# CVMI-Lab/DODA

Measured on AMD Instinct MI355X. Metric: active-voxels/sec fwd+bwd SparseConv U-Net, ScanNet 2cm, higher is better.
Workload: dtype bf16; 1 GPU; cfgs/scannet SparseConv U-Net training step (voxel pooling + fwd + CE + bwd + SGD), 2 cm voxels, 4 scenes/GPU x ~150000 active voxels, random-init weights; global_batch=4, voxels_per_gpu=601279, points_per_gpu=781042, parallelism=dp1, n_classes=20, grad_sync=deferred multi-layer wgrad + bucketed all-reduce, collectives=none (single process), prefetch_gate=off, grad_exchange=no process group

## Files before the change

### doda_amd/csrc/spconv_wgrad.hip

```cpp
#include "wgrad_pairs.hpp"
#include <stdlib.h>
#include <string.h>
#include <mutex>
#include <vector>

typedef float f32x4 __attribute__((ext_vector_type(4)));
typedef short s16x4 __attribute__((ext_vector_type(4)));
typedef __bf16 bf16x8 __attribute__((ext_vector_type(8)));
typedef unsigned int u32x4 __attribute__((ext_vector_type(4)));

namespace {

constexpr int RT = 64;
constexpr int MAX_OGW = 7;
constexpr int PAD = 8;

struct F32 {
    typedef float elem;
    typedef f32x4 frag;
    typedef f32x4 vec;
    static constexpr int VEC = 4;
    static constexpr int KSTEPS = RT / 4;
    typedef float kfrag;
    template <int STRIDE>
// ... 374 lines not shown
    const dim3 grid(total_blocks), block(256);
#define GO(TA, TB, OG)                                                                             \
    do {                                                                                           \
        if (vok) hipLaunchKernelGGL((wgrad_multi_kernel<T, TA, TB, OG, true>), grid, block, 0, s, jobs_dev, n); \
        else hipLaunchKernelGGL((wgrad_multi_kernel<T, TA, TB, OG, false>), grid, block, 0, s, jobs_dev, n); \
    } while (0)
    if (p.OGW == 2) {
        if (p.TA == 3 && p.TB == 3) GO(3, 3, 2);
        else if (p.TA == 1 && p.TB == 1) GO(1, 1, 2);
        else if (p.TA == 2 && p.TB == 1) GO(2, 1, 2);
        else if (p.TA == 1 && p.TB == 2) GO(1, 2, 2);
        else GO(2, 2, 2);
    } else if (p.OGW == 4 && p.TA == 1 && p.TB == 1) GO(1, 1, 4);
    else if (p.OGW == 4 && p.TA == 2 && p.TB == 1) GO(2, 1, 4);
    else if (p.OGW == 4 && p.TA == 1 && p.TB == 2) GO(1, 2, 4);
    else if (p.TA == 1 && p.TB == 1) GO(1, 1, 7);
    else if (p.TA == 2 && p.TB == 1) GO(2, 1, 7);
    else if (p.TA == 1 && p.TB == 2) GO(1, 2, 7);
    else GO(2, 2, 4);
#undef GO
}

struct Staging {
    std::mutex mu;
    void *host = nullptr;
    size_t cap = 0;
    hipEvent_t ev = nullptr;
    int ev_dev = -1;
    bool pending = false;
};
Staging g_staging;
}

enum { J_SKIP = 0, J_ZERO = 1, J_DENSE = 2, J_PAIRS = 3, J_TILE = 4 };

static int wdma_min_rows() {
    static const int v = getenv("DODA_WDMA_MIN_ROWS") ? atoi(getenv("DODA_WDMA_MIN_ROWS")) : 32768;
    return v;
}

static int classify(const doda_wgrad_job &j) {
    if (j.n_rows == 0 && j.dw && j.K > 0 && j.ca > 0 && j.cb > 0)
        return (j.flags & DODA_WGRAD_ACCUMULATE) ? J_SKIP : J_ZERO;
    if (j.tilebook && j.tbl && j.elem_bytes == 2 && j.ca % 16 == 0 && j.ca <= 64 && j.cb % 16 == 0 && j.cb <= 64 &&
        j.K == 27 && j.n_rows > 0 && j.a && j.b && j.dw &&
        j.n_a == j.n_rows && j.ld >= j.n_rows && (size_t)j.n_rows * 128 < 0x7ffffff0ull && (size_t)j.K * j.ld * 4 < 0xffffffffull &&
        !(((uintptr_t)j.a | (uintptr_t)j.b | (uintptr_t)j.tilebook) & 15) && doda_wdma::enabled() &&
        (j.n_rows >= wdma_min_rows() || !doda_pairs::eligible(j)))
        return J_TILE;
    static const bool no_pairs = getenv("DODA_WGRAD_NO_PAIRS") && getenv("DODA_WGRAD_NO_PAIRS")[0] == '1';
    if (doda_pairs::eligible(j) && (!no_pairs || !j.tbl)) return J_PAIRS;
    return J_DENSE;
}

static size_t tile_blocks(const doda_wgrad_job &j) { return (size_t)(j.ca / 16) * (j.cb / 16); }

static bool dense_needs_partial(const JobPlan &jp, const doda_wgrad_job &j) {
    return jp.p.R > 1 || (j.flags & DODA_WGRAD_ACCUMULATE);
}

extern "C" size_t doda_spconv_wgrad_multi_workspace_bytes(const doda_wgrad_job *jobs_h, int32_t n_jobs) {
    if (!jobs_h || n_jobs <= 0) return 0;
    size_t total = 0;
    for (int k = 0; k < n_jobs; ++k) {
        const int cls = classify(jobs_h[k]);
        if (cls == J_PAIRS) { total += doda_pairs::partial_bytes(jobs_h[k]); continue; }
        if (cls == J_TILE) { total += tile_blocks(jobs_h[k]) * align_up(doda_wdma::partial_bytes(jobs_h[k].n_rows), 256); continue; }
        if (cls != J_DENSE) continue;
        JobPlan jp;
        if (!plan_job(jobs_h[k], &jp)) continue;
        if (dense_needs_partial(jp, jobs_h[k])) total += align_up((size_t)jp.p.R * jp.n_elem * 4, 256);
    }
    return total < 256 ? 256 : total;
}

extern "C" size_t doda_spconv_wgrad_multi_desc_bytes(int32_t n_jobs) {
    const size_t per = sizeof(WJob) + sizeof(RJob) > doda_pairs::desc_bytes_per_job()
                           ? sizeof(WJob) + sizeof(RJob) : doda_pairs::desc_bytes_per_job();
    return n_jobs <= 0 ? 0 : align_up((size_t)n_jobs * per + 256, 256);
}

extern "C" int doda_spconv_wgrad_multi(const doda_wgrad_job *jobs_h, int32_t n_jobs, void *ws, size_t ws_bytes,
                                       void *desc_dev, size_t desc_bytes, doda_stream_t stream) {
    if (!jobs_h || n_jobs <= 0 || !ws || !desc_dev) return DODA_ERR_INVALID;
    if (desc_bytes < doda_spconv_wgrad_multi_desc_bytes(n_jobs)) return DODA_ERR_WORKSPACE;
    hipStream_t s = as_stream(stream);
    std::vector<JobPlan> plans(n_jobs);
    std::vector<int> keys, cls(n_jobs), pair_jobs, tile_jobs;
    size_t off = 0;
    for (int k = 0; k < n_jobs; ++k) {
        plans[k].key = -1;
        cls[k] = classify(jobs_h[k]);
        if (cls[k] == J_ZERO) {
            hipMemsetAsync(jobs_h[k].dw, 0, (size_t)jobs_h[k].K * jobs_h[k].ca * jobs_h[k].cb * 4, s);
            continue;
        }
        if (cls[k] == J_SKIP) continue;
        if (cls[k] == J_PAIRS) { pair_jobs.push_back(k); continue; }
        if (cls[k] == J_TILE) { tile_jobs.push_back(k); continue; }
        if (!plan_job(jobs_h[k], &plans[k])) return DODA_ERR_INVALID;
        plans[k].ws_off = off;
        if (dense_needs_partial(plans[k], jobs_h[k])) off += align_up((size_t)plans[k].p.R * plans[k].n_elem * 4, 256);
        bool seen = false;
        for (int key : keys) seen |= key == plans[k].key;
        if (!seen) keys.push_back(plans[k].key);
    }
    doda_pairs::Prepared prep;
    if (!pair_jobs.empty()) {
        const int st = doda_pairs::prepare(jobs_h, pair_jobs.data(), (int)pair_jobs.size(), (char *)ws, &off, &prep);
        if (st != DODA_OK) return st;
    }
    {
        std::vector<char> done(tile_jobs.size(), 0);
        for (size_t q = 0; q < tile_jobs.size(); ++q) {
            if (done[q]) continue;
            const doda_wgrad_job &j0 = jobs_h[tile_jobs[q]];
            std::vector<doda_wdma::Block> blocks;
            for (size_t r = q; r < tile_jobs.size(); ++r) {
                const doda_wgrad_job &j = jobs_h[tile_jobs[r]];
                if (done[r] || j.tilebook != j0.tilebook || j.tbl != j0.tbl || j.n_rows != j0.n_rows || j.ld != j0.ld) continue;
                done[r] = 1;
                const int es = 2;
                for (int ci = 0; ci < j.ca; ci += 16)
                    for (int co = 0; co < j.cb; co += 16)
                        blocks.push_back(doda_wdma::Block{(const char *)j.a + ci * es, (const char *)j.b + co * es,
                                                          j.dw + (size_t)ci * j.cb + co, j.ca * es, j.cb * es, j.ca * j.cb, j.cb,
                                                          (j.flags & DODA_WGRAD_ACCUMULATE) ? 1 : 0});
            }
            const size_t bytes = blocks.size() * align_up(doda_wdma::partial_bytes(j0.n_rows), 256);
            if (ws_bytes < off + bytes) return DODA_ERR_WORKSPACE;
            const int st = doda_wdma::launch(blocks.data(), (int)blocks.size(), j0.tbl, j0.ld, j0.n_rows, j0.tilebook,
                                             (char *)ws + off, s);
            if (st != DODA_OK) return st;
            off += bytes;
        }
    }
    if (ws_bytes < off) return DODA_ERR_WORKSPACE;

    std::vector<WJob> wj;
    std::vector<RJob> rj;
    struct Group { int first, count, blocks, rep; };
    std::vector<Group> groups;
    for (int key : keys) {
        Group g{(int)wj.size(), 0, 0, -1};
        for (int k = 0; k < n_jobs; ++k) {
            if (cls[k] != J_DENSE || plans[k].key != key) continue;
            const doda_wgrad_job &j = jobs_h[k];
            const Plan &p = plans[k].p;
            if (g.rep < 0) g.rep = k;
            WJob d;
            d.a = j.a; d.b = j.b; d.tbl = j.tbl;
            d.out = dense_needs_partial(plans[k], j) ? (float *)((char *)ws + plans[k].ws_off) : j.dw;
            d.ca = j.ca; d.cb = j.cb; d.ld = j.ld; d.K = j.K; d.n_rows = j.n_rows;
            d.rows_per_chunk = p.rows_per_chunk; d.n_tag = p.n_tag; d.n_tbg = p.n_tbg; d.n_og = p.n_og;
            g.blocks += p.R * p.n_tag * p.n_tbg * p.n_og;
            d.blk_end = g.blocks;
            wj.push_back(d);
            ++g.count;
        }
        groups.push_back(g);
    }
    int r_blocks = 0;
    bool scalar_reduce = false;
    for (int k = 0; k < n_jobs; ++k) {
        if (cls[k] != J_DENSE || !dense_needs_partial(plans[k], jobs_h[k])) continue;
        if (plans[k].n_elem % 4 != 0 || (uintptr_t)jobs_h[k].dw % 16 != 0) { scalar_reduce = true; continue; }
        RJob d;
        d.partial = (const float4 *)((char *)ws + plans[k].ws_off);
        d.dw = (float4 *)jobs_h[k].dw;
        d.n_quad = plans[k].n_elem / 4;
        d.R = plans[k].p.R;
        d.accumulate = (jobs_h[k].flags & DODA_WGRAD_ACCUMULATE) ? 1 : 0;
        d.pad = 0;
        int rl = 1;
        while (rl < 16 && rl < d.R) rl *= 2;
        d.pad = rl;
        r_blocks += (int)div_up(d.n_quad, 256 / rl);
        d.blk_end = r_blocks;
        rj.push_back(d);
    }
    const size_t wbytes = wj.size() * sizeof(WJob), rbytes = rj.size() * sizeof(RJob);
    const size_t pair_off = align_up(wbytes + rbytes, 16), pbytes = prep.desc.size();
    const size_t total_desc = pair_off + pbytes;
    if (total_desc > desc_bytes) return DODA_ERR_WORKSPACE;
    if (total_desc > 0) {
        std::lock_guard<std::mutex> lock(g_staging.mu);
        Staging &st = g_staging;
        if (st.pending) { hipEventSynchronize(st.ev); st.pending = false; }
        if (st.cap < total_desc) {
            if (st.host) hipHostFree(st.host);
            st.cap = align_up(total_desc, 4096) * 2;
            if (hipHostMalloc(&st.host, st.cap, hipHostMallocDefault) != hipSuccess) { st.host = nullptr; st.cap = 0; return DODA_ERR_NOMEM; }
        }
        int cur_dev = 0;
        hipGetDevice(&cur_dev);
        if (st.ev && st.ev_dev != cur_dev) { hipEventDestroy(st.ev); st.ev = nullptr; }
        if (!st.ev && hipEventCreateWithFlags(&st.ev, hipEventDisableTiming) != hipSuccess) return DODA_ERR_LAUNCH;
        st.ev_dev = cur_dev;
        if (wbytes) memcpy(st.host, wj.data(), wbytes);
        if (rbytes) memcpy((char *)st.host + wbytes, rj.data(), rbytes);
        if (pbytes) memcpy((char *)st.host + pair_off, prep.desc.data(), pbytes);
        if (hipMemcpyAsync(desc_dev, st.host, total_desc, hipMemcpyHostToDevice, s) != hipSuccess) return DODA_ERR_LAUNCH;
        hipEventRecord(st.ev, s);
        st.pending = true;
    }
    const WJob *wj_dev = (const WJob *)desc_dev;
    for (const Group &g : groups) {
        const JobPlan &jp = plans[g.rep];
        if (jp.esz == 4 && jp.split) launch_multi_variant<F32S>(jp.p, jp.vok, g.blocks, wj_dev + g.first, g.count, s);
        else if (jp.esz == 4) launch_multi_variant<F32>(jp.p, jp.vok, g.blocks, wj_dev + g.first, g.count, s);
        else launch_multi_variant<BF16>(jp.p, jp.vok, g.blocks, wj_dev + g.first, g.count, s);
    }
    int st = doda_check_launch();
    if (st != DODA_OK) return st;
    if (!pair_jobs.empty()) {
        st = doda_pairs::launch(prep, (const char *)desc_dev + pair_off, s);
        if (st != DODA_OK) return st;
    }
    if (!rj.empty()) {
        hipLaunchKernelGGL(wgrad_reduce_multi, dim3(r_blocks), dim3(256), 0, s,
                           (const RJob *)((const char *)desc_dev + wbytes), (int)rj.size());
        st = doda_check_launch();
        if (st != DODA_OK) return st;
    }
    if (scalar_reduce)
        for (int k = 0; k < n_jobs; ++k) {
            if (cls[k] != J_DENSE || !dense_needs_partial(plans[k], jobs_h[k])) continue;
            if (plans[k].n_elem % 4 == 0 && (uintptr_t)jobs_h[k].dw % 16 == 0) continue;
            hipLaunchKernelGGL(wgrad_reduce, dim3(div_up(plans[k].n_elem, 16)), dim3(256), 0, s,
                               (const float *)((char *)ws + plans[k].ws_off), plans[k].p.R, plans[k].n_elem,
                               jobs_h[k].dw, (jobs_h[k].flags & DODA_WGRAD_ACCUMULATE) ? 1 : 0);
        }
    return doda_check_launch();
}
```

### doda_amd/csrc/wgrad_pairs.hpp

```cpp
#pragma once
#include "common.hpp"
#include <vector>

namespace doda_pairs {

bool eligible(const doda_wgrad_job &j);

size_t partial_bytes(const doda_wgrad_job &j);

struct Prepared {
    std::vector<unsigned char> desc;
    struct Group { int ta, tb, first, count, blocks; };
    std::vector<Group> groups;
    size_t reduce_off = 0;
    int n_reduce = 0, reduce_blocks = 0;
};

int prepare(const doda_wgrad_job *jobs, const int *which, int n, char *ws_base, size_t *ws_off, Prepared *out);

int launch(const Prepared &p, const void *desc_dev, hipStream_t s);

size_t desc_bytes_per_job();

}

namespace doda_wdma {
bool enabled();
void set_enabled(bool on);
int max_jobs();
size_t partial_bytes(int n_rows);
struct Block { const void *x, *dy; float *dw; int x_stride, dy_stride, ldo, ldc, accumulate; };
int launch(const Block *blocks, int n_blocks, const int32_t *tbl, int ld, int n_rows, const void *tilebook, void *part,
           hipStream_t s);
}
```

### doda_amd/csrc_ext/doda_torch.cpp

```cpp
#include <torch/extension.h>
#include <torch/csrc/autograd/engine.h>
#include <torch/csrc/autograd/function.h>
#include <torch/csrc/autograd/functions/utils.h>
#include <torch/csrc/autograd/graph_task.h>
#include <torch/csrc/autograd/saved_variable.h>
#include <c10/hip/HIPGuard.h>
#include <unordered_map>
#include <c10/hip/HIPStream.h>
#include <c10/hip/HIPCachingAllocator.h>
#include <hip/hip_runtime_api.h>

#include <cstring>
#include <functional>
#include <mutex>
#include <vector>

#include "../../include/doda_hip.h"
#include <chrono>
#include <cstdlib>

static const bool g_poison = [] { const char *e = getenv("DODA_POISON"); return e && e[0] == '1'; }();
static inline at::Tensor poisoned(at::Tensor t) {
    if (g_poison && t.defined() && t.is_cuda() && t.numel() > 0)
        (void)hipMemsetAsync(t.data_ptr(), 0xFF, (size_t)t.numel() * t.element_size(), c10::hip::getCurrentHIPStream(t.device().index()).stream());
// ... 274 lines not shown
}

bool read_back_blocking(const void *dev_ptr, int32_t *out, int n, void *st, int dev) {
    static const bool spin = getenv("DODA_SPIN_READBACK") && getenv("DODA_SPIN_READBACK")[0] == '1';
    if (spin) return false;
    struct Slot { int32_t *host = nullptr; hipEvent_t ev = nullptr; int dev = -1; };
    static thread_local Slot slot;
    const int cur = dev;
    c10::hip::HIPGuard dev_guard((c10::DeviceIndex)dev);
    if (!slot.host)
        TORCH_CHECK(hipHostMalloc((void **)&slot.host, 64, hipHostMallocDefault) == hipSuccess, "doda: hipHostMalloc");
    if (!slot.ev || slot.dev != cur) {
        if (slot.ev) (void)hipEventDestroy(slot.ev);
        slot.ev = nullptr;
        TORCH_CHECK(hipEventCreateWithFlags(&slot.ev, hipEventBlockingSync | hipEventDisableTiming) == hipSuccess, "doda: hipEventCreate");
        slot.dev = cur;
    }
    TORCH_CHECK(hipMemcpyAsync(slot.host, dev_ptr, (size_t)n * 4, hipMemcpyDeviceToHost, (hipStream_t)st) == hipSuccess, "doda: hipMemcpyAsync");
    TORCH_CHECK(hipEventRecord(slot.ev, (hipStream_t)st) == hipSuccess, "doda: hipEventRecord");
    TORCH_CHECK(hipEventSynchronize(slot.ev) == hipSuccess, "doda: hipEventSynchronize");
    for (int k = 0; k < n; ++k) out[k] = slot.host[k];
    return true;
}
int32_t read_back_i32(const at::Tensor &t, void *st) {
    int32_t v = 0;
    if (read_back_blocking(t.data_ptr(), &v, 1, st, (int)t.device().index())) return v;
    return t.item<int32_t>();
}

typedef std::tuple<at::Tensor, at::Tensor, at::Tensor, at::Tensor, std::vector<int64_t>, at::Tensor, at::Tensor,
                   at::Tensor, at::Tensor, at::Tensor, at::Tensor> PyramidLevel;
std::vector<PyramidLevel> build_pyramid(const at::Tensor &indices_in, std::vector<int64_t> shape, int64_t batch,
                                        int64_t n_levels, int64_t pairs_min_rows, int64_t tile_min_rows,
                                        int64_t tile_levels) {
    TORCH_CHECK(indices_in.is_cuda() && indices_in.scalar_type() == at::kInt && indices_in.dim() == 2 &&
                indices_in.size(1) == 4 && shape.size() == 3, "doda build_pyramid: indices must be int32 [M,4] on the GPU");
    std::vector<PyramidLevel> out;
    at::Tensor indices = indices_in.contiguous();
    const auto iopt = indices.options();
    void *st = stream_of(indices);
    for (int64_t lvl = 0; lvl < n_levels; ++lvl) {
        const int32_t m = (int32_t)indices.size(0);
        int32_t shp[3] = {(int32_t)shape[0], (int32_t)shape[1], (int32_t)shape[2]};
        size_t wsb = doda_rulebook_workspace_bytes(m);
        {
            const long double cells = (long double)batch * shape[0] * shape[1] * shape[2];
            static const long long grid_max = [] {
                const char *e = getenv("DODA_RULEBOOK_GRID_MAX_LOG2");
                const int b = e ? atoi(e) : 28;
                return 1ll << (b < 0 ? 0 : b > 30 ? 30 : b);
            }();
            if (m > 0 && cells > 0 && cells <= (long double)grid_max) wsb = (wsb + 255) / 256 * 256 + (size_t)cells * 4;
        }
        at::Tensor ws = pempty({(int64_t)(wsb > 256 ? wsb : 256)}, iopt.dtype(at::kByte));
        const bool tiled = lvl < tile_levels && tile_min_rows >= 0 && m >= tile_min_rows;
        at::Tensor nbr = tiled ? table_with_tilebook(27, m, iopt) : pempty({27, m}, iopt);
        check(doda_rulebook_subm((const int32_t *)indices.data_ptr(), m, shp, (int32_t)batch, 3,
                                 (int32_t *)nbr.data_ptr(), m, ws.data_ptr(), (size_t)ws.numel(), st),
              "doda_rulebook_subm");
        if (tiled) build_tilebook(nbr, st);
        at::Tensor sp, sn, sh, dp, dn, dh;
        const bool with_pairs = pairs_min_rows >= 0 && m >= pairs_min_rows;
        const bool subm_pairs = with_pairs && !tiled;
        if (subm_pairs) std::tie(sp, sn, sh) = export_pairs(nbr, m, true, st);
        if (lvl == n_levels - 1) {
            out.emplace_back(nbr, at::Tensor(), at::Tensor(), at::Tensor(), std::vector<int64_t>(), sp, sn, sh, dp, dn, dh);
            break;
        }
        at::Tensor parent = pempty({m > 0 ? m : 1}, iopt), off = pempty({m > 0 ? m : 1}, iopt);
        at::Tensor out_idx = pempty({m > 0 ? m : 1, 4}, iopt), count = pempty({1}, iopt);
        check(doda_rulebook_down2_assign((const int32_t *)indices.data_ptr(), m, shp, (int32_t)batch,
                                         (int32_t *)parent.data_ptr(), (int32_t *)off.data_ptr(),
                                         (int32_t *)out_idx.data_ptr(), (int32_t *)count.data_ptr(), ws.data_ptr(),
                                         (size_t)ws.numel(), st), "doda_rulebook_down2_assign");
        const int32_t m_out = read_back_i32(count, st);
        at::Tensor child = pempty({8, m_out}, iopt), par_off = pempty({8, m}, iopt);
        check(doda_rulebook_down2_tables((const int32_t *)parent.data_ptr(), (const int32_t *)off.data_ptr(), m, m_out,
                                         (int32_t *)child.data_ptr(), m_out, (int32_t *)par_off.data_ptr(), m, st),
              "doda_rulebook_down2_tables");
        static const bool down_pairs = [] { const char *e = getenv("DODA_WGRAD_PAIRS_DOWN"); return e && e[0] == '1'; }();
        if (with_pairs && down_pairs) std::tie(dp, dn, dh) = export_pairs(par_off, m, false, st);
        std::vector<int64_t> oshape = {(shape[0] - 2) / 2 + 1, (shape[1] - 2) / 2 + 1, (shape[2] - 2) / 2 + 1};
        at::Tensor outids = out_idx.narrow(0, 0, m_out);
        out.emplace_back(nbr, outids, child, par_off, oshape, sp, sn, sh, dp, dn, dh);
        indices = outids;
        shape = oshape;
    }
    return out;
// ... 1261 lines not shown
                                  pair_in, pair_out, pair_num, pair_seg, true);
        return std::make_pair(r[0], r[1].defined() ? c10::optional<at::Tensor>(r[1]) : c10::nullopt);
    }, "sparse conv that also returns the BatchNorm statistics partials of its output",
          py::arg("features"), py::arg("weight"), py::arg("fwd_tbl"), py::arg("bwd_tbl"), py::arg("n_out"),
          py::arg("bwd_layout"), py::arg("pk_fwd"), py::arg("pk_bwd"), py::arg("residual"),
          py::arg("pair_in") = py::none(), py::arg("pair_out") = py::none(), py::arg("pair_num") = py::none(),
          py::arg("pair_seg") = py::none());
    m.def("residual_block", [](const at::Tensor &x, const c10::optional<at::Tensor> &stats_in, const std::vector<at::Tensor> &bn1,
                               const std::vector<at::Tensor> &bn2, bool training, double momentum1, double eps1,
                               double momentum2, double eps2, const std::vector<c10::optional<at::Tensor>> &cv1,
                               const std::vector<c10::optional<at::Tensor>> &cv2,
                               const std::vector<c10::optional<at::Tensor>> &rb, int64_t n_out,
                               const c10::optional<at::Tensor> &skip, bool want_stats,
                               const std::vector<c10::optional<at::Tensor>> &sc, const c10::optional<at::Tensor> &stats_in_b) {
        auto r = residual_block(x, stats_in, bn1, bn2, training, momentum1, eps1, momentum2, eps2, cv1, cv2, rb, n_out, skip,
                                want_stats, sc, stats_in_b);
        return std::make_pair(r[0], r[1].defined() ? c10::optional<at::Tensor>(r[1]) : c10::nullopt);
    }, "BatchNorm -> ReLU -> SubM conv -> BatchNorm -> ReLU -> SubM conv (+ skip) in one call",
          py::arg("x"), py::arg("stats_in"), py::arg("bn1"), py::arg("bn2"), py::arg("training"), py::arg("momentum1"),
          py::arg("eps1"), py::arg("momentum2"), py::arg("eps2"), py::arg("cv1"), py::arg("cv2"), py::arg("rb"),
          py::arg("n_out"), py::arg("skip"), py::arg("want_stats"),
          py::arg("sc") = std::vector<c10::optional<at::Tensor>>(), py::arg("stats_in_b") = py::none());
    m.def("set_bn_fusion", [](bool on) { g_bn_fusion = on; }, "BatchNorm statistics in the conv epilogues (default on)");
    m.def("gather", [](const at::Tensor &x, const at::Tensor &w, const c10::optional<at::Tensor> &packed,
                       const at::Tensor &tbl, int64_t n_out, int64_t layout, int64_t nc, bool out_f32) {
        return gather(x, w, packed, tbl, n_out, layout, nc, out_f32);
    }, "raw gather-GEMM");
    m.def("wgrad", [](const at::Tensor &a, const at::Tensor &b, const at::Tensor &tbl, int64_t n_rows) {
        return wgrad(a, b, tbl, n_rows);
    }, "raw weight gradient");
    m.def("build_pyramid", &build_pyramid,
          "all SubM k3 and k2s2 rulebooks of an n-level U-Net in one call (13 native builds, 6 size read-backs)",
          py::arg("indices"), py::arg("shape"), py::arg("batch"), py::arg("n_levels"), py::arg("pairs_min_rows") = -1,
          py::arg("tile_min_rows") = -1, py::arg("tile_levels") = 2,
          py::call_guard<py::gil_scoped_release>());
    m.def("build_pyramid_probe", [](const at::Tensor &indices, std::vector<int64_t> shape, int64_t batch, int64_t n_levels,
                                    int64_t pairs_min_rows, int64_t tile_min_rows, int64_t tile_levels) {
              auto levels = build_pyramid(indices, shape, batch, n_levels, pairs_min_rows, tile_min_rows, tile_levels);
              int64_t nt = -1, o64 = 0, o32 = 0;
              if (!levels.empty()) {
                  const at::Tensor &tbl = std::get<0>(levels[0]);
                  const void *tb = tilebook_behind(tbl, tbl.dim() == 2 ? tbl.size(1) : 0);
                  if (tb) {
                      const int64_t T = doda_tilebook_tile(), K = tbl.size(0), UMAX = doda_tilebook_umax();
                      nt = (tbl.size(1) + T - 1) / T;
                      (void)K; (void)UMAX; (void)nt;
                      char *p = (char *)const_cast<void *>(tb) + doda_tilebook_bytes((int32_t)tbl.size(1), (int32_t)tbl.size(0)) - 8;
                      int32_t ov[2] = {0, 0};
                      if (!read_back_blocking(p, ov, 2, stream_of(tbl), (int)tbl.device().index())) {
                          at::Tensor over = at::from_blob(p, {2}, tbl.options()).cpu();
                          ov[0] = over[0].item<int32_t>();
                          ov[1] = over[1].item<int32_t>();
                      }
                      o64 = ov[0];
                      o32 = ov[1];
                  }
              }
              return std::make_tuple(levels, nt, o64, o32);
          }, py::arg("indices"), py::arg("shape"), py::arg("batch"), py::arg("n_levels"), py::arg("pairs_min_rows") = -1,
          py::arg("tile_min_rows") = -1, py::arg("tile_levels") = 2, py::call_guard<py::gil_scoped_release>());
    m.def("with_tilebook", [](const at::Tensor &tbl) {
              TORCH_CHECK(tbl.is_cuda() && tbl.scalar_type() == at::kInt && tbl.dim() == 2, "doda with_tilebook: int32 [K, M] table");
              at::Tensor out = table_with_tilebook(tbl.size(0), tbl.size(1), tbl.options());
              out.copy_(tbl);
              if (tilebook_behind(out, out.size(1))) build_tilebook(out, stream_of(out));
              return out;
          }, "copy of a gather table with its tilebook (doda_tilebook_build) in the same storage");
    m.def("has_tilebook", [](const at::Tensor &tbl) { return tilebook_behind(tbl, tbl.dim() == 2 ? tbl.size(1) : 0) != nullptr; });
    m.def("tilebook_parts", [](const at::Tensor &tbl) {
              const void *tb = tilebook_behind(tbl, tbl.size(1));
              TORCH_CHECK(tb, "doda tilebook_parts: no tilebook");
              const int64_t T = doda_tilebook_tile(), nt = (tbl.size(1) + T - 1) / T, K = tbl.size(0), UMAX = doda_tilebook_umax();
              TORCH_CHECK(K == 27 && T == 256, "doda tilebook_parts: layout of csrc/tilebook.hpp");
              const int64_t LW = 10;
              char *p = (char *)const_cast<void *>(tb);
              auto o32 = tbl.options();
              at::Tensor order = pempty({UMAX}, at::TensorOptions().dtype(at::kLong));
              for (int64_t e = 0; e < UMAX; ++e) order.data_ptr<int64_t>()[e] = (((e >> 5) & 7) * 32 + (e & 31)) * 4 + (e >> 8);
              at::Tensor ulist = at::from_blob(p, {nt, UMAX}, o32).index_select(1, order.to(tbl.device()));
              at::Tensor pos = pempty({T}, at::TensorOptions().dtype(at::kLong));
              for (int64_t t = 0; t < T; ++t) pos.data_ptr<int64_t>()[t] = (t & 0xC0) | (((t & 3) | ((t & 4) << 1) | ((t & 8) >> 1)) << 2) | ((t >> 4) & 3);
              at::Tensor words = at::from_blob(p + nt * UMAX * 4, {nt, LW, T}, o32).to(at::kLong).index_select(2, pos.to(tbl.device()));
              std::vector<at::Tensor> per_offset;
              for (int64_t o = 0; o < K; ++o)
                  per_offset.push_back(words.select(1, (o & 1) * 5 + (o >> 1) / 3).bitwise_right_shift(10 * ((o >> 1) % 3)).bitwise_and(0x3ff));
              at::Tensor lidx = at::stack(per_offset, 1).to(at::kShort);
              at::Tensor ucount = at::from_blob(p + nt * UMAX * 4 + nt * T * LW * 4, {nt}, o32).clone();
              return std::make_tuple(ulist, lidx, ucount);
          });
    m.def("tilebook_overflow", [](const at::Tensor &tbl) {
              const void *tb = tilebook_behind(tbl, tbl.size(1));
              TORCH_CHECK(tb, "doda tilebook_overflow: no tilebook");
              const int64_t T = doda_tilebook_tile(), nt = (tbl.size(1) + T - 1) / T, K = tbl.size(0), UMAX = doda_tilebook_umax();
// ... 86 lines not shown
```

### doda_amd/spconv/ops.py

```python
import os

import numpy as np

import torch

from .. import ops as _ops
from .._ext import ext as _ext
from .core import IndiceData

PAIRS_MIN_ROWS = 65536
WGRAD_PAIRS_DOWN = os.environ.get("DODA_WGRAD_PAIRS_DOWN", "0") == "1"


def _triple(v):
    if isinstance(v, (list, tuple, np.ndarray)):
        out = [int(x) for x in v]
        if len(out) != 3:
            raise ValueError("expected 3 values, got %r" % (v,))
        return out
    return [int(v)] * 3


def get_conv_output_size(input_size, kernel_size, stride, padding, dilation):
    out = []
# ... 11 lines not shown
        tbl = _ops.rulebook_subm(indices, spatial_shape, batch_size, k[0])
    else:
        tbl = _ops.rulebook_subm_generic(indices, spatial_shape, batch_size, k)
    return IndiceData("subm", indices, indices, list(spatial_shape), list(spatial_shape), tbl)


def build_down2(indices, batch_size, spatial_shape, ksize, stride, padding, dilation):
    k, s, p, d = _triple(ksize), _triple(stride), _triple(padding), _triple(dilation)
    if k != [2, 2, 2] or s != [2, 2, 2] or p != [0, 0, 0] or d != [1, 1, 1]:
        if k[0] * k[1] * k[2] > 27:
            raise NotImplementedError("doda_amd SparseConv3d supports kernel volumes <= 27, got k=%r" % (k,))
        outids, tbl, tbl_rev, out_shape = _ops.rulebook_conv(indices, spatial_shape, batch_size, k, s, p, d)
        return IndiceData("down2", outids, indices, list(spatial_shape), out_shape, tbl, tbl_rev)
    outids, child, par_off, out_shape = _ops.rulebook_down2(indices, spatial_shape, batch_size)
    return IndiceData("down2", outids, indices, list(spatial_shape), out_shape, child, par_off)


def get_indice_pairs(indices, batch_size, spatial_shape, ksize=3, stride=1, padding=0, dilation=1,
                     out_padding=0, subm=False, transpose=False, grid=None, use_hash=False):
    if transpose:
        raise NotImplementedError("transposed sparse convolution is not part of DODA's path")
    if subm:
        data = build_subm(indices, batch_size, spatial_shape, ksize)
    else:
        data = build_down2(indices, batch_size, spatial_shape, ksize, stride, padding, dilation)
    return data.outids, data.indice_pairs, data.indice_pair_num


TILE_MIN_ROWS = 32768
TILE_KERNEL = os.environ.get("DODA_NO_TILE", "0") != "1"
TILE_OVERFLOW_MAX = 0.25
TILE_BACKOFF = 64
_tile_state = {"skip": 0, "last": None}


def build_pyramid(tensor, n_levels, subm_key="subm%d", down_key="spconv%d", first_level=1, with_pairs=False,
                  with_tiles=None):
    indices, shape = tensor.indices, tensor.spatial_shape
    n_tile_levels = (2 if with_pairs else 0) if with_tiles is None else (2 if with_tiles is True else int(with_tiles))
    if (_ext is not None and not tensor.indice_dict and indices.is_cuda and indices.dtype == torch.int32
            and indices.shape[0] > 0 and all(int(v) >= 2 for v in shape)):
        tiles_on = TILE_KERNEL and n_tile_levels > 0
        if tiles_on and _tile_state["skip"] > 0:
            _tile_state["skip"] -= 1
            tiles_on = False
        levels, nt, over64, over32 = _ext.build_pyramid_probe(indices, [int(v) for v in shape], int(tensor.batch_size),
                                                              int(n_levels), PAIRS_MIN_ROWS if with_pairs else -1,
                                                              TILE_MIN_ROWS if tiles_on else -1, n_tile_levels)
        if tiles_on and nt >= 0:
            _tile_state["last"] = (nt, over64, over32)
            if over32 > TILE_OVERFLOW_MAX * nt:
                _tile_state["skip"] = TILE_BACKOFF
                levels = [((lv[0].clone() if _ext.has_tilebook(lv[0]) else lv[0]),) + tuple(lv[1:]) for lv in levels]
        for k, (nbr, outids, child, par_off, oshape, sp, sn, sh, dp, dn, dh) in enumerate(levels):
            lvl = first_level + k
            data = tensor.indice_dict[subm_key % lvl] = IndiceData("subm", indices, indices, list(shape),
                                                                   list(shape), nbr)
            if sp is not None:
                data._wpairs = (sp, sn, sh)
            if k == len(levels) - 1:
                break
            data = tensor.indice_dict[down_key % lvl] = IndiceData("down2", outids, indices, list(shape),
                                                                   list(oshape), child, par_off)
            if dp is not None:
                data._wpairs = (dp, dn, dh)
            indices, shape = outids, list(oshape)
        return tensor.indice_dict
    for lvl in range(first_level, first_level + n_levels):
        key = subm_key % lvl
        if key not in tensor.indice_dict:
            tensor.indice_dict[key] = build_subm(indices, tensor.batch_size, shape, 3)
        if (with_pairs and indices.shape[0] >= PAIRS_MIN_ROWS
                and not (_ext is not None and _ext.has_tilebook(tensor.indice_dict[key].tbl))):
            tensor.indice_dict[key].wgrad_lists()
        if lvl == first_level + n_levels - 1:
            break
        key = down_key % lvl
        data = tensor.indice_dict.get(key)
        if data is None:
            data = build_down2(indices, tensor.batch_size, shape, 2, 2, 0, 1)
            tensor.indice_dict[key] = data
        if with_pairs and WGRAD_PAIRS_DOWN and indices.shape[0] >= PAIRS_MIN_ROWS:
            data.wgrad_lists()
        indices, shape = data.outids, data.out_spatial_shape
    return tensor.indice_dict
```

Measured before the change: 132.9 million voxels/s.

## Add wide-channel tilebook weight-gradient kernel for deeper U-Net levels

Adds a new wgrad path (J_WIDE) for subm layers with wider channels that are not pair-eligible. It uses 1024-thread workgroups that stage dy and gathered x rows per 256-row tile in LDS, run all 27 offsets across 16 waves with bf16 MFMA, write per-chunk partials, and reduce them in a second kernel. The pyramid builder now also attaches tilebooks to deeper levels (default up to 7) so these layers can use the tile-list gather instead of the dense per-offset path. Building extra tilebooks costs more time during rulebook construction, and the partial buffers plus the separate reduce launch add memory traffic.

```diff
diff --git a/doda_amd/csrc/spconv_wgrad.hip b/doda_amd/csrc/spconv_wgrad.hip
--- a/doda_amd/csrc/spconv_wgrad.hip
+++ b/doda_amd/csrc/spconv_wgrad.hip
@@ -430,7 +430,7 @@
 Staging g_staging;
 }
 
-enum { J_SKIP = 0, J_ZERO = 1, J_DENSE = 2, J_PAIRS = 3, J_TILE = 4 };
+enum { J_SKIP = 0, J_ZERO = 1, J_DENSE = 2, J_PAIRS = 3, J_TILE = 4, J_WIDE = 5 };
 
 static int wdma_min_rows() {
     static const int v = getenv("DODA_WDMA_MIN_ROWS") ? atoi(getenv("DODA_WDMA_MIN_ROWS")) : 32768;
@@ -440,6 +440,7 @@
 static int classify(const doda_wgrad_job &j) {
     if (j.n_rows == 0 && j.dw && j.K > 0 && j.ca > 0 && j.cb > 0)
         return (j.flags & DODA_WGRAD_ACCUMULATE) ? J_SKIP : J_ZERO;
+    if (doda_wwide::eligible(j) && !doda_pairs::eligible(j)) return J_WIDE;
     if (j.tilebook && j.tbl && j.elem_bytes == 2 && j.ca % 16 == 0 && j.ca <= 64 && j.cb % 16 == 0 && j.cb <= 64 &&
         j.K == 27 && j.n_rows > 0 && j.a && j.b && j.dw &&
         j.n_a == j.n_rows && j.ld >= j.n_rows && (size_t)j.n_rows * 128 < 0x7ffffff0ull && (size_t)j.K * j.ld * 4 < 0xffffffffull &&
@@ -451,6 +452,12 @@
     return J_DENSE;
 }
 
+static std::vector<int> wide_chunks(const doda_wgrad_job *jobs_h, const std::vector<int> &idx) {
+    std::vector<int> rpc;
+    for (int k : idx) rpc.push_back(make_plan(jobs_h[k].K, jobs_h[k].ca, jobs_h[k].cb, jobs_h[k].n_rows, 2, true).rows_per_chunk);
+    return rpc;
+}
+
 static size_t tile_blocks(const doda_wgrad_job &j) { return (size_t)(j.ca / 16) * (j.cb / 16); }
 
 static bool dense_needs_partial(const JobPlan &jp, const doda_wgrad_job &j) {
@@ -460,8 +467,10 @@
 extern "C" size_t doda_spconv_wgrad_multi_workspace_bytes(const doda_wgrad_job *jobs_h, int32_t n_jobs) {
     if (!jobs_h || n_jobs <= 0) return 0;
     size_t total = 0;
+    std::vector<int> wide_jobs;
     for (int k = 0; k < n_jobs; ++k) {
         const int cls = classify(jobs_h[k]);
+        if (cls == J_WIDE) { wide_jobs.push_back(k); continue; }
         if (cls == J_PAIRS) { total += doda_pairs::partial_bytes(jobs_h[k]); continue; }
         if (cls == J_TILE) { total += tile_blocks(jobs_h[k]) * align_up(doda_wdma::partial_bytes(jobs_h[k].n_rows), 256); continue; }
         if (cls != J_DENSE) continue;
@@ -469,12 +478,15 @@
         if (!plan_job(jobs_h[k], &jp)) continue;
         if (dense_needs_partial(jp, jobs_h[k])) total += align_up((size_t)jp.p.R * jp.n_elem * 4, 256);
     }
+    const std::vector<int> rpc = wide_chunks(jobs_h, wide_jobs);
+    total += doda_wwide::partial_bytes(jobs_h, wide_jobs.data(), rpc.data(), (int)wide_jobs.size());
     return total < 256 ? 256 : total;
 }
 
 extern "C" size_t doda_spconv_wgrad_multi_desc_bytes(int32_t n_jobs) {
-    const size_t per = sizeof(WJob) + sizeof(RJob) > doda_pairs::desc_bytes_per_job()
-                           ? sizeof(WJob) + sizeof(RJob) : doda_pairs::desc_bytes_per_job();
+    size_t per = sizeof(WJob) + sizeof(RJob) > doda_pairs::desc_bytes_per_job()
+                     ? sizeof(WJob) + sizeof(RJob) : doda_pairs::desc_bytes_per_job();
+    if (per < doda_wwide::desc_bytes_per_job()) per = doda_wwide::desc_bytes_per_job();
     return n_jobs <= 0 ? 0 : align_up((size_t)n_jobs * per + 256, 256);
 }
 
@@ -484,7 +496,7 @@
     if (desc_bytes < doda_spconv_wgrad_multi_desc_bytes(n_jobs)) return DODA_ERR_WORKSPACE;
     hipStream_t s = as_stream(stream);
     std::vector<JobPlan> plans(n_jobs);
-    std::vector<int> keys, cls(n_jobs), pair_jobs, tile_jobs;
+    std::vector<int> keys, cls(n_jobs), pair_jobs, tile_jobs, wide_jobs;
     size_t off = 0;
     for (int k = 0; k < n_jobs; ++k) {
         plans[k].key = -1;
@@ -496,6 +508,7 @@
         if (cls[k] == J_SKIP) continue;
         if (cls[k] == J_PAIRS) { pair_jobs.push_back(k); continue; }
         if (cls[k] == J_TILE) { tile_jobs.push_back(k); continue; }
+        if (cls[k] == J_WIDE) { wide_jobs.push_back(k); continue; }
         if (!plan_job(jobs_h[k], &plans[k])) return DODA_ERR_INVALID;
         plans[k].ws_off = off;
         if (dense_needs_partial(plans[k], jobs_h[k])) off += align_up((size_t)plans[k].p.R * plans[k].n_elem * 4, 256);
@@ -533,6 +546,16 @@
             off += bytes;
         }
     }
+    std::vector<unsigned char> wide_desc;
+    int wide_wgs = 0, wide_red = 0;
+    if (!wide_jobs.empty()) {
+        const std::vector<int> rpc = wide_chunks(jobs_h, wide_jobs);
+        const size_t bytes = doda_wwide::partial_bytes(jobs_h, wide_jobs.data(), rpc.data(), (int)wide_jobs.size());
+        if (ws_bytes < off + bytes) return DODA_ERR_WORKSPACE;
+        doda_wwide::prepare(jobs_h, wide_jobs.data(), rpc.data(), (int)wide_jobs.size(), (char *)ws + off, wide_desc, &wide_wgs,
+                            &wide_red);
+        off += bytes;
+    }
     if (ws_bytes < off) return DODA_ERR_WORKSPACE;
 
     std::vector<WJob> wj;
@@ -579,7 +602,8 @@
     }
     const size_t wbytes = wj.size() * sizeof(WJob), rbytes = rj.size() * sizeof(RJob);
     const size_t pair_off = align_up(wbytes + rbytes, 16), pbytes = prep.desc.size();
-    const size_t total_desc = pair_off + pbytes;
+    const size_t wide_off = align_up(pair_off + pbytes, 16), wdbytes = wide_desc.size();
+    const size_t total_desc = wide_off + wdbytes;
     if (total_desc > desc_bytes) return DODA_ERR_WORKSPACE;
     if (total_desc > 0) {
         std::lock_guard<std::mutex> lock(g_staging.mu);
@@ -598,6 +622,7 @@
         if (wbytes) memcpy(st.host, wj.data(), wbytes);
         if (rbytes) memcpy((char *)st.host + wbytes, rj.data(), rbytes);
         if (pbytes) memcpy((char *)st.host + pair_off, prep.desc.data(), pbytes);
+        if (wdbytes) memcpy((char *)st.host + wide_off, wide_desc.data(), wdbytes);
         if (hipMemcpyAsync(desc_dev, st.host, total_desc, hipMemcpyHostToDevice, s) != hipSuccess) return DODA_ERR_LAUNCH;
         hipEventRecord(st.ev, s);
         st.pending = true;
@@ -613,6 +638,10 @@
     if (st != DODA_OK) return st;
     if (!pair_jobs.empty()) {
         st = doda_pairs::launch(prep, (const char *)desc_dev + pair_off, s);
+        if (st != DODA_OK) return st;
+    }
+    if (!wide_jobs.empty()) {
+        st = doda_wwide::launch((const char *)desc_dev + wide_off, (int)wide_jobs.size(), wide_wgs, wide_red, s);
         if (st != DODA_OK) return st;
     }
     if (!rj.empty()) {
diff --git a/doda_amd/csrc/spconv_wwide.hip b/doda_amd/csrc/spconv_wwide.hip
--- /dev/null
+++ b/doda_amd/csrc/spconv_wwide.hip
@@ -0,0 +1,313 @@
+#include "common.hpp"
+#include "tilebook.hpp"
+#include "wgrad_pairs.hpp"
+#include <stdlib.h>
+#include <string.h>
+#include <algorithm>
+#include <vector>
+
+namespace {
+
+typedef float f32x4w __attribute__((ext_vector_type(4)));
+typedef short s16x4w __attribute__((ext_vector_type(4)));
+typedef __bf16 bf16x8w __attribute__((ext_vector_type(8)));
+typedef unsigned int u32x4w __attribute__((ext_vector_type(4)));
+
+constexpr int WW_WAVES = 16;
+constexpr int WW_MO = (TB_K + WW_WAVES - 1) / WW_WAVES;
+constexpr int WW_MAX_BLOCKS = 9;
+constexpr int WW_MAX_TA = 3, WW_MAX_TB = 7;
+constexpr int WW_LIST_BYTES = TB_UMAX * 4;
+constexpr int ww_stage_bytes(int ta, int tb) { return TB_T * 32 * tb + (TB_LMAX + 1) * 32 * ta; }
+constexpr int WW_STAGE_MAX = ww_stage_bytes(3, 3);
+constexpr int WW_SMEM = WW_LIST_BYTES + TB_LIDX_BYTES + WW_STAGE_MAX;
+static_assert(WW_SMEM <= 160 * 1024, "one workgroup per CU");
+static_assert(TB_T + 1 <= TB_LMAX + 1, "the dense fallback stages 256 rows into the row slots");
+
+struct WwJob {
+    const unsigned short *x, *dy;
+    const int32_t *tbl;
+    const void *tb;
+    float *dw, *part;
+    int ca, cb, ld, n_rows, nt, ta, tb_, n_sb, P, rpc, accumulate;
+    int wg_end, red_end;
+    int pad;
+};
+
+template <class J>
+__device__ __forceinline__ int ww_find(const J *jobs, int n, int blk, bool red) {
+    int lo = 0, hi = n - 1;
+    while (lo < hi) {
+        const int mid = (lo + hi) >> 1;
+        if (blk < (red ? jobs[mid].red_end : jobs[mid].wg_end)) hi = mid; else lo = mid + 1;
+    }
+    return lo;
+}
+
+__device__ __forceinline__ s16x4w ww_tr(unsigned addr) {
+    return __builtin_amdgcn_ds_read_tr16_b64_v4i16((__attribute__((address_space(3))) s16x4w *)(uintptr_t)addr);
+}
+__device__ __forceinline__ bf16x8w ww_frag(unsigned a_lo, unsigned a_hi) {
+    const s16x4w lo = ww_tr(a_lo), hi = ww_tr(a_hi);
+    return __builtin_bit_cast(bf16x8w, __builtin_shufflevector(lo, hi, 0, 1, 2, 3, 4, 5, 6, 7));
+}
+
+template <int TA, int TB>
+__device__ void ww_body(const WwJob &d, int local, unsigned char *smem) {
+    constexpr int RA = 32 * TA, RB = 32 * TB;
+    constexpr int CIS = 16 * TA, COS = 16 * TB, SLICE = TB_K * CIS * COS;
+    const int tid = threadIdx.x, wid = __builtin_amdgcn_readfirstlane(tid >> 6);
+    const int lane = tid & 63, i = lane & 15, g = lane >> 4, q4 = i >> 2, c4 = i & 3;
+    const int slice = local / d.P, p = local - slice * d.P;
+    const int sa = slice / d.n_sb, sb = slice - sa * d.n_sb;
+    const int ca0 = sa * CIS, cb0 = sb * COS;
+    const int r_begin = p * d.rpc, r_end = min(d.n_rows, r_begin + d.rpc);
+    const int tile_begin = r_begin / TB_T, tile_end = (r_end - 1) / TB_T + 1;
+    static_assert(ww_stage_bytes(TA, TB) <= WW_STAGE_MAX, "staging buffers");
+    const int32_t *tb_ulist = (const int32_t *)d.tb;
+    const uint32_t *tb_lidx = (const uint32_t *)(tb_ulist + (size_t)d.nt * TB_UMAX);
+    const int32_t *tb_ucount = (const int32_t *)(tb_lidx + (size_t)d.nt * (TB_LIDX_BYTES / 4));
+
+    int32_t *list_s = reinterpret_cast<int32_t *>(smem);
+    const unsigned *lidx_s = reinterpret_cast<const unsigned *>(smem + WW_LIST_BYTES);
+    unsigned char *dy_s = smem + WW_LIST_BYTES + TB_LIDX_BYTES;
+    unsigned char *rows_s = dy_s + TB_T * RB;
+    const unsigned dy_base = (unsigned)(uintptr_t)dy_s, rows_base = (unsigned)(uintptr_t)rows_s;
+
+    f32x4w acc[WW_MO][TA][TB];
+#pragma unroll
+    for (int m = 0; m < WW_MO; ++m)
+#pragma unroll
+        for (int a = 0; a < TA; ++a)
+#pragma unroll
+            for (int b = 0; b < TB; ++b) acc[m][a][b] = (f32x4w){0.f, 0.f, 0.f, 0.f};
+
+    auto multiply = [&](bool dense, int only_o, int ks_begin, int ks_end) {
+#pragma unroll 1
+        for (int ks = ks_begin; ks < ks_end; ++ks) {
+            const int r = 32 * ks + 8 * g + q4;
+            bf16x8w bf[TB];
+#pragma unroll
+            for (int b = 0; b < TB; ++b) {
+                const unsigned a0 = dy_base + (unsigned)(r * RB + b * 32 + c4 * 8);
+                bf[b] = ww_frag(a0, a0 + 4u * RB);
+            }
+#pragma unroll
+            for (int m = 0; m < WW_MO; ++m) {
+                const int o = wid + WW_WAVES * m;
+                if (o >= TB_K || (dense && o != only_o)) continue;
+                unsigned s0, s1;
+                if (dense) {
+                    s0 = (unsigned)(r + 1);
+                    s1 = (unsigned)(r + 5);
+                } else {
+                    const unsigned *pl = lidx_s + tb_lplane(o) * TB_T;
+                    const unsigned sh = tb_lshift(o);
+                    s0 = __builtin_amdgcn_ubfe(pl[tb_lpos(r)], sh, 10u);
+                    s1 = __builtin_amdgcn_ubfe(pl[tb_lpos(r + 4)], sh, 10u);
+                }
+                const unsigned x0 = rows_base + s0 * RA + (unsigned)(c4 * 8), x1 = rows_base + s1 * RA + (unsigned)(c4 * 8);
+#pragma unroll
+                for (int a = 0; a < TA; ++a) {
+                    const bf16x8w af = ww_frag(x0 + 32u * a, x1 + 32u * a);
+#pragma unroll
+                    for (int b = 0; b < TB; ++b)
+                        acc[m][a][b] = __builtin_amdgcn_mfma_f32_16x16x32_bf16(af, bf[b], acc[m][a][b], 0, 0, 0);
+                }
+            }
+        }
+    };
+
+    for (int e = tid; e < RA / 16; e += 1024) reinterpret_cast<u32x4w *>(rows_s)[e] = (u32x4w){0u, 0u, 0u, 0u};
+    for (int tile = tile_begin; tile < tile_end; ++tile) {
+        const int t0 = tile * TB_T;
+        const int ks_begin = max(0, (r_begin - t0) / 32), ks_end = min(TB_T / 32, (r_end - t0 + 31) / 32);
+        const int ucount = tb_ucount[tile];
+        const bool listed = ucount <= TB_LMAX;
+        if (listed) {
+            const int e = (tid & 3) * 256 + ((tid >> 7) & 7) * 32 + ((tid >> 2) & 31);
+            list_s[e] = tb_ulist[(size_t)tile * TB_UMAX + tid];
+            for (int v = tid; v < TB_LIDX_BYTES / 16; v += 1024)
+                reinterpret_cast<u32x4w *>(smem + WW_LIST_BYTES)[v] =
+                    reinterpret_cast<const u32x4w *>(tb_lidx + (size_t)tile * (TB_LIDX_BYTES / 4))[v];
+        }
+        for (int v = tid; v < TB_T * (RB / 16); v += 1024) {
+            const int t = v / (RB / 16), f = v - t * (RB / 16);
+            u32x4w val = (u32x4w){0u, 0u, 0u, 0u};
+            if (t0 + t < d.n_rows) val = *reinterpret_cast<const u32x4w *>(d.dy + (size_t)(t0 + t) * d.cb + cb0 + f * 8);
+            *reinterpret_cast<u32x4w *>(dy_s + t * RB + f * 16) = val;
+        }
+        doda_sync();
+        if (listed) {
+            for (int v = tid; v < ucount * (RA / 16); v += 1024) {
+                const int e = v / (RA / 16), f = v - e * (RA / 16);
+                const int row = list_s[e];
+                *reinterpret_cast<u32x4w *>(rows_s + (e + 1) * RA + f * 16) =
+                    *reinterpret_cast<const u32x4w *>(d.x + (size_t)row * d.ca + ca0 + f * 8);
+            }
+            doda_sync();
+            multiply(false, 0, ks_begin, ks_end);
+            doda_sync();
+        } else {
+            for (int o = 0; o < TB_K; ++o) {
+                for (int v = tid; v < TB_T * (RA / 16); v += 1024) {
+                    const int t = v / (RA / 16), f = v - t * (RA / 16);
+                    const int row = t0 + t < d.n_rows ? d.tbl[(size_t)o * d.ld + t0 + t] : -1;
+                    u32x4w val = (u32x4w){0u, 0u, 0u, 0u};
+                    if (row >= 0) val = *reinterpret_cast<const u32x4w *>(d.x + (size_t)row * d.ca + ca0 + f * 8);
+                    *reinterpret_cast<u32x4w *>(rows_s + (t + 1) * RA + f * 16) = val;
+                }
+                doda_sync();
+                multiply(true, o, ks_begin, ks_end);
+                doda_sync();
+            }
+        }
+    }
+
+    float *dst = d.part + (size_t)local * SLICE;
+#pragma unroll
+    for (int m = 0; m < WW_MO; ++m) {
+        const int o = wid + WW_WAVES * m;
+        if (o >= TB_K) continue;
+#pragma unroll
+        for (int a = 0; a < TA; ++a)
+#pragma unroll
+            for (int b = 0; b < TB; ++b)
+#pragma unroll
+                for (int r = 0; r < 4; ++r)
+                    dst[((size_t)o * CIS + a * 16 + 4 * g + r) * COS + b * 16 + i] = acc[m][a][b][r];
+    }
+}
+
+#define WW_SHAPES(X) X(3, 3) X(2, 4) X(2, 3) X(1, 5) X(1, 6) X(1, 7) X(1, 4) X(1, 3)
+
+__global__ __launch_bounds__(1024) void wgrad_wide(const WwJob *__restrict__ jobs, int n_jobs) {
+    __shared__ __attribute__((aligned(16))) unsigned char smem[WW_SMEM];
+    const int j = ww_find(jobs, n_jobs, (int)blockIdx.x, false);
+    const WwJob d = jobs[j];
+    const int local = (int)blockIdx.x - (j == 0 ? 0 : jobs[j - 1].wg_end);
+#define WW_CASE(A, B) if (d.ta == A && d.tb_ == B) { ww_body<A, B>(d, local, smem); return; }
+    WW_SHAPES(WW_CASE)
+#undef WW_CASE
+}
+
+__global__ __launch_bounds__(256) void wgrad_wide_reduce(const WwJob *__restrict__ jobs, int n_jobs) {
+    __shared__ float4 part[256];
+    const int j = ww_find(jobs, n_jobs, (int)blockIdx.x, true);
+    const WwJob d = jobs[j];
+    const int blk = (int)blockIdx.x - (j == 0 ? 0 : jobs[j - 1].red_end);
+    int RL = 1;
+    while (RL < 16 && RL < d.P) RL *= 2;
+    const int EL = 256 / RL, el = (int)threadIdx.x % EL, rl = (int)threadIdx.x / EL;
+    const long long q = (long long)blk * EL + el, n_quad = (long long)TB_K * d.ca * d.cb / 4;
+    const int CIS = 16 * d.ta, COS = 16 * d.tb_, SLICE = TB_K * CIS * COS;
+    const float *src = nullptr;
+    if (q < n_quad) {
+        const long long e = 4 * q;
+        const int co = (int)(e % d.cb), ci = (int)((e / d.cb) % d.ca), o = (int)(e / ((long long)d.ca * d.cb));
+        const int slice = (ci / CIS) * d.n_sb + co / COS;
+        src = d.part + ((size_t)slice * d.P) * SLICE + ((size_t)o * CIS + ci % CIS) * COS + co % COS;
+    }
+    float4 s = make_float4(0.f, 0.f, 0.f, 0.f);
+    if (src)
+        for (int r = rl; r < d.P; r += RL) {
+            const float4 v = *reinterpret_cast<const float4 *>(src + (size_t)r * SLICE);
+            s.x += v.x; s.y += v.y; s.z += v.z; s.w += v.w;
+        }
+    part[rl * EL + el] = s;
+    doda_sync();
+    if (rl == 0 && src) {
+        float4 t = part[el];
+        for (int r = 1; r < RL; ++r) {
+            const float4 v = part[r * EL + el];
+            t.x += v.x; t.y += v.y; t.z += v.z; t.w += v.w;
+        }
+        float4 *dst = reinterpret_cast<float4 *>(d.dw) + q;
+        if (d.accumulate) {
+            const float4 old = *dst;
+            t.x += old.x; t.y += old.y; t.z += old.z; t.w += old.w;
+        }
+        *dst = t;
+    }
+}
+
+bool ww_shape(int ca, int cb, int *ta, int *tb) {
+    const int A = ca / 16, B = cb / 16;
+    int b = B;
+    while (b > WW_MAX_TB || B % b) --b;
+    int a = WW_MAX_TA;
+    while (a > 1 && (A % a || a * b > WW_MAX_BLOCKS)) --a;
+    bool known = false;
+#define WW_KNOWN(X, Y) known |= (a == X && b == Y);
+    WW_SHAPES(WW_KNOWN)
+#undef WW_KNOWN
+    *ta = a; *tb = b;
+    return known;
+}
+
+}
+
+namespace doda_wwide {
+
+bool eligible(const doda_wgrad_job &j) {
+    int ta, tb;
+    return j.tilebook && j.tbl && j.elem_bytes == 2 && j.K == TB_K && j.n_rows > 0 && j.a && j.b && j.dw &&
+           j.ca % 16 == 0 && j.cb % 16 == 0 && j.ca >= 48 && j.cb >= 48 && j.ca <= 224 && j.cb <= 224 &&
+           j.n_a == j.n_rows && j.ld >= j.n_rows && !(((uintptr_t)j.a | (uintptr_t)j.b | (uintptr_t)j.tilebook | (uintptr_t)j.dw) & 15) &&
+           ww_shape(j.ca, j.cb, &ta, &tb);
+}
+
+struct Plan { std::vector<int> order; std::vector<WwJob> d; int wgs = 0, red_blocks = 0; size_t part_bytes = 0; };
+
+static Plan plan(const doda_wgrad_job *jobs, const int *idx, const int *rows_per_chunk, int n) {
+    Plan pl;
+    for (int k = 0; k < n; ++k) pl.order.push_back(k);
+    std::stable_sort(pl.order.begin(), pl.order.end(), [&](int a, int b) { return jobs[idx[a]].n_rows > jobs[idx[b]].n_rows; });
+    for (int kk : pl.order) {
+        const doda_wgrad_job &j = jobs[idx[kk]];
+        WwJob d;
+        d.x = (const unsigned short *)j.a; d.dy = (const unsigned short *)j.b; d.tbl = j.tbl; d.tb = j.tilebook;
+        d.dw = j.dw; d.part = nullptr;
+        d.ca = j.ca; d.cb = j.cb; d.ld = j.ld; d.n_rows = j.n_rows; d.nt = (j.n_rows + TB_T - 1) / TB_T;
+        ww_shape(j.ca, j.cb, &d.ta, &d.tb_);
+        d.n_sb = j.cb / (16 * d.tb_);
+        d.rpc = rows_per_chunk[kk];
+        d.P = (j.n_rows + d.rpc - 1) / d.rpc;
+        d.accumulate = (j.flags & DODA_WGRAD_ACCUMULATE) ? 1 : 0;
+        const int slices = (j.ca / (16 * d.ta)) * d.n_sb;
+        d.part = (float *)(uintptr_t)pl.part_bytes;
+        pl.part_bytes += align_up((size_t)slices * d.P * TB_K * 256 * d.ta * d.tb_ * 4, 256);
+        pl.wgs += slices * d.P;
+        d.wg_end = pl.wgs;
+        int rl = 1;
+        while (rl < 16 && rl < d.P) rl *= 2;
+        pl.red_blocks += (int)div_up((long long)TB_K * j.ca * j.cb / 4, 256 / rl);
+        d.red_end = pl.red_blocks;
+        d.pad = 0;
+        pl.d.push_back(d);
+    }
+    return pl;
+}
+
+size_t partial_bytes(const doda_wgrad_job *jobs, const int *idx, const int *rows_per_chunk, int n) {
+    return n ? plan(jobs, idx, rows_per_chunk, n).part_bytes : 0;
+}
+size_t desc_bytes_per_job() { return sizeof(WwJob); }
+
+void prepare(const doda_wgrad_job *jobs, const int *idx, const int *rows_per_chunk, int n, void *part,
+             std::vector<unsigned char> &desc, int *wgs, int *red_blocks) {
+    Plan pl = plan(jobs, idx, rows_per_chunk, n);
+    for (WwJob &d : pl.d) d.part = (float *)((char *)part + (uintptr_t)d.part);
+    desc.resize(pl.d.size() * sizeof(WwJob));
+    memcpy(desc.data(), pl.d.data(), desc.size());
+    *wgs = pl.wgs;
+    *red_blocks = pl.red_blocks;
+}
+
+int launch(const void *desc_dev, int n, int wgs, int red_blocks, hipStream_t s) {
+    hipLaunchKernelGGL(wgrad_wide, dim3(wgs), dim3(1024), 0, s, (const WwJob *)desc_dev, n);
+    hipLaunchKernelGGL(wgrad_wide_reduce, dim3(red_blocks), dim3(256), 0, s, (const WwJob *)desc_dev, n);
+    return doda_check_launch();
+}
+
+}
diff --git a/doda_amd/csrc/wgrad_pairs.hpp b/doda_amd/csrc/wgrad_pairs.hpp
--- a/doda_amd/csrc/wgrad_pairs.hpp
+++ b/doda_amd/csrc/wgrad_pairs.hpp
@@ -33,3 +33,12 @@
 int launch(const Block *blocks, int n_blocks, const int32_t *tbl, int ld, int n_rows, const void *tilebook, void *part,
            hipStream_t s);
 }
+
+namespace doda_wwide {
+bool eligible(const doda_wgrad_job &j);
+size_t partial_bytes(const doda_wgrad_job *jobs, const int *idx, const int *rows_per_chunk, int n);
+size_t desc_bytes_per_job();
+void prepare(const doda_wgrad_job *jobs, const int *idx, const int *rows_per_chunk, int n, void *part,
+             std::vector<unsigned char> &desc, int *wgs, int *red_blocks);
+int launch(const void *desc_dev, int n, int wgs, int red_blocks, hipStream_t s);
+}
diff --git a/doda_amd/csrc_ext/doda_torch.cpp b/doda_amd/csrc_ext/doda_torch.cpp
--- a/doda_amd/csrc_ext/doda_torch.cpp
+++ b/doda_amd/csrc_ext/doda_torch.cpp
@@ -330,7 +330,7 @@
                    at::Tensor, at::Tensor, at::Tensor, at::Tensor> PyramidLevel;
 std::vector<PyramidLevel> build_pyramid(const at::Tensor &indices_in, std::vector<int64_t> shape, int64_t batch,
                                         int64_t n_levels, int64_t pairs_min_rows, int64_t tile_min_rows,
-                                        int64_t tile_levels) {
+                                        int64_t tile_levels, int64_t wgrad_tile_levels) {
     TORCH_CHECK(indices_in.is_cuda() && indices_in.scalar_type() == at::kInt && indices_in.dim() == 2 &&
                 indices_in.size(1) == 4 && shape.size() == 3, "doda build_pyramid: indices must be int32 [M,4] on the GPU");
     std::vector<PyramidLevel> out;
@@ -351,7 +351,8 @@
             if (m > 0 && cells > 0 && cells <= (long double)grid_max) wsb = (wsb + 255) / 256 * 256 + (size_t)cells * 4;
         }
         at::Tensor ws = pempty({(int64_t)(wsb > 256 ? wsb : 256)}, iopt.dtype(at::kByte));
-        const bool tiled = lvl < tile_levels && tile_min_rows >= 0 && m >= tile_min_rows;
+        const bool tiled = (lvl < tile_levels && tile_min_rows >= 0 && m >= tile_min_rows) ||
+                           (lvl >= tile_levels && lvl < wgrad_tile_levels && m > 0 && !(pairs_min_rows >= 0 && m >= pairs_min_rows));
         at::Tensor nbr = tiled ? table_with_tilebook(27, m, iopt) : pempty({27, m}, iopt);
         check(doda_rulebook_subm((const int32_t *)indices.data_ptr(), m, shp, (int32_t)batch, 3,
                                  (int32_t *)nbr.data_ptr(), m, ws.data_ptr(), (size_t)ws.numel(), st),
@@ -1679,11 +1680,13 @@
     m.def("build_pyramid", &build_pyramid,
           "all SubM k3 and k2s2 rulebooks of an n-level U-Net in one call (13 native builds, 6 size read-backs)",
           py::arg("indices"), py::arg("shape"), py::arg("batch"), py::arg("n_levels"), py::arg("pairs_min_rows") = -1,
-          py::arg("tile_min_rows") = -1, py::arg("tile_levels") = 2,
+          py::arg("tile_min_rows") = -1, py::arg("tile_levels") = 2, py::arg("wgrad_tile_levels") = 0,
           py::call_guard<py::gil_scoped_release>());
     m.def("build_pyramid_probe", [](const at::Tensor &indices, std::vector<int64_t> shape, int64_t batch, int64_t n_levels,
-                                    int64_t pairs_min_rows, int64_t tile_min_rows, int64_t tile_levels) {
-              auto levels = build_pyramid(indices, shape, batch, n_levels, pairs_min_rows, tile_min_rows, tile_levels);
+                                    int64_t pairs_min_rows, int64_t tile_min_rows, int64_t tile_levels,
+                                    int64_t wgrad_tile_levels) {
+              auto levels = build_pyramid(indices, shape, batch, n_levels, pairs_min_rows, tile_min_rows, tile_levels,
+                                          wgrad_tile_levels);
               int64_t nt = -1, o64 = 0, o32 = 0;
               if (!levels.empty()) {
                   const at::Tensor &tbl = std::get<0>(levels[0]);
@@ -1705,7 +1708,8 @@
               }
               return std::make_tuple(levels, nt, o64, o32);
           }, py::arg("indices"), py::arg("shape"), py::arg("batch"), py::arg("n_levels"), py::arg("pairs_min_rows") = -1,
-          py::arg("tile_min_rows") = -1, py::arg("tile_levels") = 2, py::call_guard<py::gil_scoped_release>());
+          py::arg("tile_min_rows") = -1, py::arg("tile_levels") = 2, py::arg("wgrad_tile_levels") = 0,
+          py::call_guard<py::gil_scoped_release>());
     m.def("with_tilebook", [](const at::Tensor &tbl) {
               TORCH_CHECK(tbl.is_cuda() && tbl.scalar_type() == at::kInt && tbl.dim() == 2, "doda with_tilebook: int32 [K, M] table");
               at::Tensor out = table_with_tilebook(tbl.size(0), tbl.size(1), tbl.options());
diff --git a/doda_amd/spconv/ops.py b/doda_amd/spconv/ops.py
--- a/doda_amd/spconv/ops.py
+++ b/doda_amd/spconv/ops.py
@@ -67,6 +67,7 @@
 TILE_OVERFLOW_MAX = 0.25
 TILE_BACKOFF = 64
 _tile_state = {"skip": 0, "last": None}
+WGRAD_TILE_LEVELS = int(os.environ.get("DODA_WGRAD_TILE_LEVELS", "7"))
 
 
 def build_pyramid(tensor, n_levels, subm_key="subm%d", down_key="spconv%d", first_level=1, with_pairs=False,
@@ -81,12 +82,14 @@
             tiles_on = False
         levels, nt, over64, over32 = _ext.build_pyramid_probe(indices, [int(v) for v in shape], int(tensor.batch_size),
                                                               int(n_levels), PAIRS_MIN_ROWS if with_pairs else -1,
-                                                              TILE_MIN_ROWS if tiles_on else -1, n_tile_levels)
+                                                              TILE_MIN_ROWS if tiles_on else -1, n_tile_levels,
+                                                              WGRAD_TILE_LEVELS if (with_pairs and n_tile_levels > 0) else 0)
         if tiles_on and nt >= 0:
             _tile_state["last"] = (nt, over64, over32)
             if over32 > TILE_OVERFLOW_MAX * nt:
                 _tile_state["skip"] = TILE_BACKOFF
-                levels = [((lv[0].clone() if _ext.has_tilebook(lv[0]) else lv[0]),) + tuple(lv[1:]) for lv in levels]
+                levels = [((lv[0].clone() if k < n_tile_levels and _ext.has_tilebook(lv[0]) else lv[0]),) + tuple(lv[1:])
+                          for k, lv in enumerate(levels)]
         for k, (nbr, outids, child, par_off, oshape, sp, sn, sh, dp, dn, dh) in enumerate(levels):
             lvl = first_level + k
             data = tensor.indice_dict[subm_key % lvl] = IndiceData("subm", indices, indices, list(shape),
```

Measured after the change: 138.2 million voxels/s (median of 6 runs). +4.0%, better.
